# TheShadow29/zsgnet-pytorch

Measured on AMD Instinct MI355X. Metric: train images/sec, higher is better.
Workload: dtype f32

## Files before the change

### zsgnet-pytorch_amd/csrc/common.h

```cpp
#pragma once
#include <hip/hip_runtime.h>
#include <hip/hip_ext.h>
#include <stdint.h>
#include <stdio.h>
#include <string.h>

#include "zsg.h"

typedef float f32x4 __attribute__((ext_vector_type(4)));
typedef float f32x16 __attribute__((ext_vector_type(16)));

struct BnbDev {
    const float* x;
    const float* mean;
    const float* invstd;
    const unsigned char* mask;
    int store_masked;
};

int zsg_conv_pw_launch(const zsg_conv_desc* d, int uw, const float* src, const float* wt, float* out, const float* bias, const float* add_src,
                       const float* mask_src, float* bn_partials, const BnbDev* bnb, hipStream_t st);

bool zsg_conv_mx_ok(const zsg_conv_desc* d, const char** why);
int zsg_conv_mx_groups(const zsg_conv_desc* d);
int zsg_conv_mx_launch(const zsg_conv_desc* d, const float* src, const float* wt, float* out, const float* bias, const float* add_src,
                       const float* mask_src, float* bn_partials, hipStream_t st);

#ifndef ZSG_MAIN_PRIO
#define ZSG_MAIN_PRIO 3
#endif
typedef int (*zsg_prio_setter_t)(int);
void zsg_register_prio_setter(zsg_prio_setter_t fn);
#define ZSG_DEFINE_PRIO_FLAG()                                                                                                      \
    __constant__ int zsg_prio_flag_c = ZSG_MAIN_PRIO;                                                                               \
    static int zsg_prio_set_(int v) {                                                                                               \
        return hipMemcpyToSymbol(HIP_SYMBOL(zsg_prio_flag_c), &v, sizeof(int), 0, hipMemcpyHostToDevice) == hipSuccess ? 0 : -3;      \
    }                                                                                                                               \
    namespace {                                                                                                                     \
    struct ZsgPrioReg {                                                                                                             \
        ZsgPrioReg() { zsg_register_prio_setter(zsg_prio_set_); }                                                                   \
    } zsg_prio_reg_;                                                                                                                \
    }
#define ZSG_SET_MAIN_PRIO() do { if (zsg_prio_flag_c) __builtin_amdgcn_s_setprio(3); } while (0)

#define ZSG_WAVE 64
#define ZSG_NUM_CU 256
#define ZSG_NUM_XCD 8
#define ZSG_MAX_DEV 64

void zsg_set_error(const char* fmt, ...);
#define ZSG_FAIL(code, ...)          \
    do {                             \
        zsg_set_error(__VA_ARGS__);  \
        return (code);               \
    } while (0)
#define ZSG_REQUIRE(cond, ...)                   \
    do {                                         \
        if (!(cond)) ZSG_FAIL(-1, __VA_ARGS__);  \
    } while (0)
#define ZSG_CHECK_LAUNCH(name)                                                            \
    do {                                                                                  \
        hipError_t e__ = hipGetLastError();                                               \
        if (e__ != hipSuccess) ZSG_FAIL(-3, "%s: launch failed: %s", name, hipGetErrorString(e__)); \
    } while (0)

extern thread_local hipEvent_t zsg_tls_completion_event;
extern thread_local int zsg_tls_completion_uses;
#define ZSG_LAUNCH(kernel, grid, block, shmem, stream, ...)                                                                   \
    do {                                                                                                                      \
        if (zsg_tls_completion_event) {                                                                                       \
            hipExtLaunchKernelGGL(kernel, grid, block, shmem, stream, nullptr, zsg_tls_completion_event, 0, __VA_ARGS__);      \
            ++zsg_tls_completion_uses;                                                                                        \
        } else                                                                                                                  \
            hipLaunchKernelGGL(kernel, grid, block, shmem, stream, __VA_ARGS__);                                              \
    } while (0)

#define ZSG_SK_FLAG_BYTES 16384
#define ZSG_SK_ERR_WORD (ZSG_SK_FLAG_BYTES / 4 - 1)
void* zsg_stream_workspace(hipStream_t st, size_t* bytes);

struct ZsgProfScope {
    int slot;
    hipStream_t st;
    ZsgProfScope(const char* name, hipStream_t s, double flops, double bytes);
    ~ZsgProfScope();
};
extern int g_zsg_prof_on;
extern int g_zsg_deterministic;
#define ZSG_PROF(name, stream, flops, bytes) ZsgProfScope prof__(name, (hipStream_t)(stream), (flops), (bytes))

static inline double zsg_conv_alg_bytes(const zsg_conv_desc* d, bool reads_out) {
    double e = (double)d->N * d->seg[0].ty.n * d->seg[0].tx.n * d->C;
    for (int s = 0; s < d->nseg; ++s) {
        const zsg_seg& a = d->seg[s];
        e += (double)d->B * a.src_H * a.src_W * d->C + (double)d->B * a.rows_y * a.rows_x * d->N * (reads_out ? 2.0 : 1.0);
    }
    return 4.0 * e;
}

__device__ __forceinline__ float wave_sum(float v) {
#pragma unroll
    for (int o = 32; o > 0; o >>= 1) v += __shfl_xor(v, o, 64);
    return v;
}
__device__ __forceinline__ double wave_sum_d(double v) {
#pragma unroll
    for (int o = 32; o > 0; o >>= 1) v += __shfl_xor(v, o, 64);
    return v;
}
// ... 28 lines not shown
```

### zsgnet-pytorch_amd/csrc/wgrad.hip

```cpp
#include <stdlib.h>

#include "wgrad_common.h"

template <int KL>
__device__ __forceinline__ void wgrad_reduce_body(const WgReduceJob& p, int block, f32x4* sm_) {
    constexpr int EL = 256 / KL;
    f32x4 (*sm)[EL] = (f32x4 (*)[EL])sm_;
    const int q4 = p.ncols / 4;
    const int64_t total = (int64_t)p.N * q4;
    const size_t slab = (size_t)p.N * p.ncols;
    const int el = threadIdx.x % EL, kl = threadIdx.x / EL;
    const int64_t i = (int64_t)block * EL + el;
    f32x4 s = {0.f, 0.f, 0.f, 0.f};
    int n = 0, q = 0;
    if (i < total) {
        n = (int)(i / q4);
        q = (int)(i % q4) * 4;
        const float* src = p.ws + (size_t)n * p.ncols + q;
#pragma unroll 4
        for (int k = kl; k < p.splits; k += KL) s += *(const f32x4*)(src + k * slab);
    }
    sm[kl][el] = s;
    __syncthreads();
    for (int o = KL / 2; o > 0; o >>= 1) {
// ... 156 lines not shown
        for (int j = 0; j < NB; ++j) *(f32x4*)&Bs[buf][kb + PB * j][4 * gb] = rb[j];
    };

    f32x16 acc[TM][TN];
#pragma unroll
    for (int i = 0; i < TM; ++i)
#pragma unroll
        for (int j = 0; j < TN; ++j)
#pragma unroll
            for (int e = 0; e < 16; ++e) acc[i][j][e] = 0.f;

    const int n_kt = kt_end - kt_begin;
    if (n_kt > 0) {
        load_tile(ra[0], rb[0], true);
        store_tile(0, ra[0], rb[0]);
#pragma unroll
        for (int st = 0; st < NS - 1; ++st) load_tile(ra[st], rb[st], n_kt > st + 1);
    }
    __syncthreads();

    const int am = wm * (32 * TM) + TM * li;
    const int bn = wn * (32 * TN) + TN * li;
    auto k_step = [&](int it, f32x4 (&cur_a)[NA], f32x4 (&cur_b)[NB], f32x4 (&nxt_a)[NA], f32x4 (&nxt_b)[NB]) {
        const int buf = it & 1;
        load_tile(nxt_a, nxt_b, it + NS < n_kt);
        __builtin_amdgcn_sched_barrier(0);
#pragma unroll
        for (int kk = 0; kk < WG_BK / 2; ++kk) {
            const int k = 2 * kk + lh;
            float fa[TM], fb[TN];
#pragma unroll
            for (int i = 0; i < TM; ++i) fa[i] = As[buf][k][am + i];
#pragma unroll
            for (int j = 0; j < TN; ++j) fb[j] = Bs[buf][k][bn + j];
#pragma unroll
            for (int i = 0; i < TM; ++i)
#pragma unroll
                for (int j = 0; j < TN; ++j)
                    acc[i][j] = __builtin_amdgcn_mfma_f32_32x32x2f32(fa[i], fb[j], acc[i][j], 0, 0, 0);
        }
        store_tile(buf ^ 1, cur_a, cur_b);
        __syncthreads();
    };
    for (int it = 0; it < n_kt; it += NS) {
#pragma unroll
        for (int st = 0; st < NS; ++st)
            if (it + st < n_kt) k_step(it + st, ra[st], rb[st], ra[(st + NS - 1) % NS], rb[(st + NS - 1) % NS]);
    }
    if (kt_begin >= kt_end) return;

#pragma unroll
    for (int j = 0; j < TN; ++j) {
        const int qc = n0 + wn * (32 * TN) + TN * li + j;
        const bool cok = qc < p.ncols;
        size_t coff;
        if (p.ws) {
            coff = (size_t)split * p.N * p.ncols + qc;
        } else {
            const int qq = cok ? qc : 0;
            const int tapi = qq / p.C;
            const int c = qq - tapi * p.C;
            const int jy = tapi / p.txn, jx = tapi - jy * p.txn;
            const int wr = p.ty.w0 + jy * p.ty.wstep, ws_ = p.tx.w0 + jx * p.tx.wstep;
            coff = (size_t)((wr * p.wS + ws_) * p.wC + p.wc0 + c);
        }
        const int ld = p.ws ? p.ncols : p.wt_ld;
        float* dst = p.ws ? p.ws : p.dw;
#pragma unroll
        for (int i = 0; i < TM; ++i) {
#pragma unroll
            for (int e = 0; e < 16; ++e) {
                const int n = m0 + wm * (32 * TM) + TM * ((e & 3) + 8 * (e >> 2) + 4 * lh) + i;
                if (cok && n < p.N) {
                    float* o = dst + (size_t)n * ld + coff;
                    *o = (!p.ws && p.accumulate) ? *o + acc[i][j][e] : acc[i][j][e];
                }
            }
        }
    }
}

extern "C" size_t zsg_conv_wgrad_workspace_bytes(const zsg_conv_desc* d) {
    if (!d) return 0;
    int splits = (d->tile_hint >> 16) & 0xff;
    if (splits <= 0) splits = 64;
    const size_t ncols = (size_t)d->seg[0].ty.n * d->seg[0].tx.n * d->C;
    return (size_t)splits * d->N * ncols * sizeof(float);
}

static const int g_zsg_wg_no_dense = [] { const char* e = getenv("ZSG_WG_DENSE"); return (e && e[0] == '0') ? 1 : 0; }();

static int conv_wgrad_impl(const zsg_conv_desc* d, const float* src, const float* dy, float* dw, int32_t accumulate, void* ws,
                           size_t ws_bytes, void* stream) {
    ZSG_REQUIRE(d && src && dy && dw, "conv_wgrad: null argument");
    ZSG_REQUIRE(d->nseg >= 1 && d->nseg <= ZSG_MAX_SEG, "conv_wgrad: nseg=%d", d->nseg);
    ZSG_REQUIRE(d->C > 0 && (d->C % 4) == 0 && (d->src_ld % 4) == 0 && (d->wC % 4) == 0 && (d->wc0 % 4) == 0,
                "conv_wgrad: C=%d src_ld=%d wC=%d wc0=%d must be multiples of 4", d->C, d->src_ld, d->wC, d->wc0);
    WgParams p;
    memset(&p, 0, sizeof(p));
    p.src = src; p.dy = dy; p.dw = dw; p.accumulate = accumulate ? 1 : 0;
    p.C = d->C; p.N = d->N; p.src_ld = d->src_ld; p.out_ld = d->out_ld; p.wS = d->wS; p.wC = d->wC; p.wc0 = d->wc0;
    p.wt_ld = d->wt_ld; p.nseg = d->nseg;
    p.ty = d->seg[0].ty; p.tx = d->seg[0].tx;
    p.txn = p.tx.n;
    p.ncols = p.ty.n * p.tx.n * d->C;
    int kt = 0;
    double rows_all = 0;
    bool wide = false;
    const bool avec = (d->out_ld & 3) == 0;
    int BKsel = (avec && ((d->tile_hint >> 25) & 1) && ((d->tile_hint >> 8) & 0xff) != 255) ? 32 : 16;
    for (int s = 0; s < d->nseg; ++s)
        if (d->seg[s].src_bstride >= (1 << 23) || d->seg[s].out_bstride >= (1 << 23)) BKsel = 16;
    p.bk = BKsel;
    for (int s = 0; s < d->nseg; ++s) {
        const zsg_seg& a = d->seg[s];
        ZSG_REQUIRE(memcmp(&a.ty, &p.ty, sizeof(zsg_taps)) == 0 && memcmp(&a.tx, &p.tx, sizeof(zsg_taps)) == 0,
                    "conv_wgrad: segments must share one tap structure (pass the forward descriptor)");
        const int64_t rows = (int64_t)d->B * a.rows_y * a.rows_x;
        ZSG_REQUIRE(rows > 0 && rows < (1ll << 24), "conv_wgrad: seg %d rows=%lld (must be < 2^24)", s, (long long)rows);
        ZSG_REQUIRE(a.src_off + (int64_t)d->B * a.src_bstride < (1ll << 29) && a.out_off + (int64_t)d->B * a.out_bstride < (1ll << 29),
                    "conv_wgrad: tensor exceeds 2^29 elements (2 GB window)");
        ZSG_REQUIRE((a.src_off % 4) == 0 && (a.src_bstride % 4) == 0, "conv_wgrad: seg %d source not 16-byte aligned", s);
        ZSG_REQUIRE(d->src_ld < (1 << 23) && d->out_ld < (1 << 23) && (int64_t)a.src_H * a.src_W < (1 << 23) &&
                        (int64_t)(a.rows_y * a.osy + a.opy + 1) * a.out_W < (1 << 23),
                    "conv_wgrad: seg %d: a row pitch / per-image pixel count exceeds 2^23", s);
        if (a.src_bstride >= (1 << 23) || a.out_bstride >= (1 << 23)) wide = true;
        WgSegDev& o = p.seg[s];
        o.rows_y = a.rows_y; o.rows_x = a.rows_x; o.rows = (int)rows; o.kt0 = kt;
        o.src_H = a.src_H; o.src_W = a.src_W; o.sy = a.sy; o.sx = a.sx;
        o.out_W = a.out_W; o.osy = a.osy; o.osx = a.osx; o.opy = a.opy; o.opx = a.opx;
        o.src_off = (int)a.src_off; o.src_bstride = (int)a.src_bstride;
        o.out_off = (int)a.out_off; o.out_bstride = (int)a.out_bstride;
        o.inv_per = 1.0f / (float)(a.rows_y * a.rows_x);
        o.inv_rx = 1.0f / (float)a.rows_x;
        kt += cdiv(rows, BKsel);
        rows_all += (double)rows;
    }
    p.kt_total = kt;
    bool dense = avec && !wide && p.ty.n == 1 && p.tx.n == 1 && p.ty.d0 == 0 && p.tx.d0 == 0 && !g_zsg_wg_no_dense;
    for (int s = 0; s < d->nseg && dense; ++s) {
        const zsg_seg& a = d->seg[s];
        dense = a.sy == 1 && a.sx == 1 && a.osy == 1 && a.osx == 1 && a.opy == 0 && a.opx == 0 && a.rows_y == a.src_H && a.rows_x == a.src_W &&
                a.out_W == a.rows_x && a.src_bstride == (int64_t)a.src_H * a.src_W * d->src_ld &&
                a.out_bstride == (int64_t)a.rows_y * a.rows_x * d->out_ld;
    }
    int TM = (d->N > 64) ? 2 : 1;
    int TN = (p.ncols > 64) ? 2 : 1;
    int want_splits = 0, w8 = 0;
    if (d->tile_hint) {
        TM = ((d->tile_hint & 0xff) >= 128) ? 2 : 1;
        TN = (((d->tile_hint >> 8) & 0xff) >= 128) ? 2 : 1;
        if (((d->tile_hint >> 8) & 0xff) == 255 && TM == 1) TN = 4;
        want_splits = (d->tile_hint >> 16) & 0xff;
        w8 = ((d->tile_hint >> 24) & 1) && TM == 2 && TN == 2;
    }
    if (!avec || wide) { TM = 1; TN = 1; w8 = 0; }
    p.m_tiles = cdiv(d->N, 64 * TM);
    p.n_tiles = cdiv(p.ncols, 64 * TN);
    const int nmn = p.m_tiles * p.n_tiles;
    int splits = want_splits > 0 ? want_splits : (2 * ZSG_NUM_CU + nmn - 1) / nmn;
    if (splits > 64 && want_splits <= 0) splits = 64;
    if (splits > kt / 2) splits = kt / 2;
    if (splits < 1) splits = 1;
    p.kt_chunk = cdiv(kt, splits);
    p.splits = cdiv(kt, p.kt_chunk);
    if (p.splits > 1) {
        const size_t need = (size_t)p.splits * d->N * p.ncols * sizeof(float);
        if (!ws || ws_bytes < need) ZSG_FAIL(-2, "conv_wgrad: workspace too small (%zu < %zu bytes)", ws_bytes, need);
        p.ws = (float*)ws;
    }
    hipStream_t st = (hipStream_t)stream;
    int dev = 0;
    (void)hipGetDevice(&dev);
    ZSG_REQUIRE(dev >= 0 && dev < ZSG_MAX_DEV, "conv_wgrad: device %d", dev);
    const double wg_flops = 2.0 * rows_all * d->N * p.ncols;
    const double wg_bytes = zsg_conv_alg_bytes(d, accumulate != 0);
    dim3 grid(nmn * p.splits);
// ... 58 lines not shown
```

### zsgnet-pytorch_amd/mdl.py

```python
import ctypes as _ct
import math
import os
import struct as _struct
import types
import weakref
from dataclasses import dataclass, field
from typing import Any, Dict, List, Optional, Tuple

import numpy as np
import torch
from torch import nn

from . import anchors as anchors_mod
from ._lib import check, lib, require_gpu, stream_ptr
from .ops import (Level, Program, TView, WinoJobs, apply_main_priority_env, autotune_conv, autotune_wgrad_batch, conv_out, ensure_stream_scratch, dgrad_desc, fwd_desc, igemm_partial_rows, marshal,
                  shared_side_stream, tile_hint, wino_mode, wino_ok)
from .params import ParamStore, pad4, register_named

VGG_BASE = [64, 64, "M", 128, 128, "M", 256, 256, 256, "C", 512, 512, 512, "M", 512, 512, 512]
SSD_EXTRAS = [256, "S", 512, 128, "S", 256, 128, 256, 128, 256]

WGRAD_DTYPES = ("fp32", "bf16")
EVAL_TTAS = ("none", "flip")
EVAL_DTYPES = ("fp32", "bf16", "bf16_act")
# ... 1238 lines not shown
        if self.training:
            y = self.conv(L, x, name=yname or (L.name + ".y"), bn_fuse=Lb)
            return self.bn(Lb, y, relu, residual=residual, name=name)
        net = self.net
        n_w = L.cout * L.k * L.k * L.cpad
        w_off = self.fold_used
        b_off = w_off + (n_w + 3) // 4 * 4
        self.fold_used = b_off + (L.cout + 3) // 4 * 4
        assert self.fold_used <= self.fold_arena.numel(), "BN-fold arena too small"
        ents = net.store.entries
        self.fold_jobs.append((ents[L.name + ".weight"].offset, w_off, ents[Lb.name + ".weight"].offset, ents[Lb.name + ".bias"].offset,
                               b_off, self.fold_rows, L.cout, L.k * L.k * L.cpad, Lb.index))
        self.fold_rows += L.cout
        lv = x.levels[0]
        out = self.act(name or Lb.name, x.B, conv_out(lv.H, L.k, L.stride, L.pad, L.dil), conv_out(lv.W, L.k, L.stride, L.pad, L.dil), L.cout,
                       dtype=torch.float32 if L.merge_x else self.adt)
        d = fwd_desc(x, out, L.cpad, L.cout, L.k, L.stride, L.pad, L.dil, wC=L.cpad, relu=relu, merge_x=L.merge_x)
        wt, bias = self.fold_arena[w_off:w_off + n_w], self.fold_arena[b_off:b_off + L.cout]
        args = (x.buf, wt, out.buf, bias, residual.buf if residual is not None else None, None, None)
        if self._bf16_conv(d, x.buf, wt, L.cpad, 0, out.buf, bias, args[4], L.name + "+bn"):
            return out
        if x.b16 or out.b16 or (residual is not None and residual.b16):
            x32, o32, r32, finish = self._via_f32(x, out, residual)
            args = (x32.buf, wt, o32.buf, bias, r32.buf if r32 is not None else None, None, None)
            x, real_out, out = x32, out, o32
        else:
            real_out, finish = out, (lambda: None)
        wargs = None
        if wino_ok(L.k, L.stride, L.pad, L.dil) and not L.merge_x and wino_mode() != "0":
            U, job = self._wino_u(wt.data_ptr(), L.cout, L.cpad, L.k * L.k * L.cpad, L.cpad, 0)
            wargs = (x.buf, U) + args[2:]
        self._tune("igemm", lib.zsg_conv_igemm, d, args, stream_ptr(), wino_args=wargs)
        if d.use_wino:
            self.wino_jobs["fwd"].add(*job)
            self.fwd.add(lib.zsg_conv_wino, d, *wargs, what=L.name + "+bn")
        else:
            self.fwd.add(lib.zsg_conv_igemm, d, *args, what=L.name + "+bn")
        finish()
        return real_out

    def _wt(self, L: ConvL, cred: int) -> torch.Tensor:
        if L.name not in self.wt:
            n = L.cpad * L.k * L.k * cred
            off = self.wt_arena_used
            self.wt_arena_used += (n + 3) // 4 * 4
            assert self.wt_arena_used <= self.wt_arena.numel(), "dgrad weight arena too small"
            self.wt[L.name] = self.wt_arena[off:off + n]
            e = self.net.store.entries[L.name + ".weight"]
            self.wt_jobs.append((e.offset, off, L.cout, L.k * L.k, L.cpad, cred))
            check(lib.zsg_transpose_w(self.net.store.flat.data_ptr() + 4 * e.offset, self.wt[L.name].data_ptr(), L.cout, L.k * L.k, L.cpad, cred,
                                      stream_ptr()), "transpose_w")
        return self.wt[L.name]

    def _finish_prep(self):
        import struct
        if not self.wt_jobs:
            return
        blob, tile0 = b"", 0
        for (so, do, N, T, Cc, ld) in self.wt_jobs:
            tc, tn = (Cc + 63) // 64, (ld + 63) // 64
            assert Cc % 4 == 0 and ld % 4 == 0 and so % 4 == 0 and do % 4 == 0
            blob += struct.pack("<qqiiiiiiii", so, do, N, T, Cc, ld, tile0, tc, tn, 0)
            tile0 += T * tc * tn
        self.wt_jobs_dev = torch.frombuffer(bytearray(blob), dtype=torch.uint8).to(self.dev)
        self.prep.add(lib.zsg_transpose_w_batched, self.net.store.flat, self.wt_arena, self.wt_jobs_dev, len(self.wt_jobs), tile0,
                      what="transpose all dgrad weight images")
        if self.dpack_jobs:
            blob = b"".join(_struct.pack("<qqiiiiiiii", *j) for j in self.dpack_jobs)
            self.dpack_jobs_dev = torch.frombuffer(bytearray(blob), dtype=torch.uint8).to(self.dev)
            self.prep.add(lib.zsg_pack_w_bf16_batched, self.dpack_jobs_dev, len(self.dpack_jobs), self.dpack_blocks,
                          what="pack bf16 dgrad weight images")
        wj = self.wino_jobs["bwd"]
        if wj.jobs:
            self.prep.add(lib.zsg_wino_weights, wj.finish(self.dev), len(wj.jobs), wj.blocks, what="wino dgrad filter transforms")

    def _conv_rg(self, L: ConvL, src: Act) -> bool:
        return src.requires_grad or self.trains(L.name + ".weight") or (L.bias and self.trains(L.name + ".bias"))

    def _conv_bwd(self, L: ConvL, src: Act, out: Act, dy: Optional[Act] = None, completes_bn: bool = False):
        dy = dy or out.grad
        if dy is None:
            return
        if self.trains(L.name + ".weight"):
            dw = fwd_desc(src, dy, L.cpad, L.cout, L.k, L.stride, L.pad, L.dil, wC=L.cpad)
            self.wgrad(dw, src, dy, L.name + ".weight", "wgrad:" + L.name, merge_x=L.merge_x)
        if L.bias and self.trains(L.name + ".bias"):
            base = dy.levels[0].off
            self.bwd.add(lib.zsg_colsum, dy.buf[base:], 1, 0, dy.rows(), dy.ld, 0, L.cout, self.G(L.name + ".bias"), 1,
                         what="bgrad:" + L.name, lane=1)
        if src.requires_grad:
            self.dgrad(L, dy, src, n=L.cpad, completes_bn=completes_bn)

    def wgrad(self, d, src: Act, dy: Act, pname: str, what: str, merge_x: bool = False):
        gw = self.G(pname)
        args = (src.buf, dy.buf, gw, 1, self.wg_ws, self.wg_ws_bytes)
        targs = (src.buf, dy.buf, self.tune_dw, 0, self.wg_ws, self.wg_ws_bytes)
        s0 = d.seg[0]
        wino = (d.wR == 3 and d.wS == 3 and s0.sy == 1 and s0.ty.d0 == -1 and s0.ty.dstep == 1 and not d.merge_x
                and dy.ld % 4 == 0 and wino_mode() != "0")
        if self.wgrad_bf16 and self._wgrad_bf16_ok(d, merge_x):
            self._tune("wgrad", lib.zsg_conv_wgrad_bf16, d, targs, stream_ptr(), self.wg_ws_bytes)
            self.bwd.add(lib.zsg_conv_wgrad_bf16, d, *args, what=what + "+bf16", lane=1)
            self._wg_log.append((len(self.bwd.calls) - 1, d, src, dy, gw, pname, what + "+bf16"))
            return
        self._tune("wgrad", lib.zsg_conv_wgrad, d, targs, stream_ptr(), self.wg_ws_bytes, wino_args=targs if wino else None)
        self.bwd.add(lib.zsg_conv_wgrad_wino if d.use_wino else lib.zsg_conv_wgrad, d, *args, what=what, lane=1)
        self._wg_log.append((len(self.bwd.calls) - 1, d, src, dy, gw, pname, what))

    @staticmethod
    def _wgrad_bf16_ok(d, merge_x: bool = False) -> bool:
        dq = type(d).from_buffer_copy(d)
        dq.merge_x = int(bool(merge_x))
        return bool(lib.zsg_conv_wgrad_bf16_supported(_ct.byref(dq)))

    def dgrad(self, L: ConvL, dy: Act, src: Act, n: int, row0: int = 0, dx: Optional[Act] = None, completes_bn: bool = False):
        cred = dy.ld
        assert cred % 4 == 0
        wt = self._wt(L, cred)
        dx = dx or self.grad_of(src)
        d = dgrad_desc(dy, dx, cred, n, L.k, L.stride, L.pad, L.dil)
        wt_off = row0 * L.k * L.k * cred
        if d.zero_fill and not dx.gfilled:
            (self.prep if self._side_prep else self.bwd).add(lib.zsg_memset_f32, self.base(dx), sum(dx.B * l.H * l.W * dx.ld for l in dx.levels), 0.0,
                                                             what="zero:" + L.name)
            dx.gfilled = True
        mask = None
        if src.needs_mask:
            deltas = {sl.off - dl.off for sl, dl in zip(src.levels, dx.levels)}
            assert len(deltas) == 1 and src.ld == dx.ld, "ReLU mask needs one common offset between src and its gradient"
            mask = src.buf.data_ptr() + 4 * deltas.pop()
            self.bwd.keep.append(src.buf)
        if self._b16_eligible(L.name) and not getattr(src, "bn_out", False) and lib.zsg_conv_igemm_bf16_m_supported(_ct.byref(d)):
            key = (L.name, row0, n)
            if key not in self._dpack:
                self._dpack[key], job, nblk = self._pack_image(wt.data_ptr() + 4 * wt_off, n, L.k * L.k, cred, 0, cred)
                self.dpack_jobs.append(job + (self.dpack_blocks, 0))
                self.dpack_blocks += nblk
            add = dx if dx.gfilled else None
            args = (dy.buf, self._dpack[key], dx.buf, None, dx.buf if dx.gfilled else None, mask)
            self._tune("igemm", lib.zsg_conv_igemm_bf16_m, d, args, stream_ptr())
            self.bwd.add(lib.zsg_conv_igemm_bf16_m, d, *args, what="dgrad:" + L.name + "+bf16")
            self._b16_log.append(dict(kind="dgrad", what="dgrad:" + L.name, idx=-1, call=self.bwd.calls[-1], d=type(d).from_buffer_copy(d),
                                      src=dy, out=dx, add=add, mask=src if mask is not None else None, pname=L.name + ".weight",
                                      window=(row0, n)))
            dx.gfilled = True
            dx.last_writer = None
            return
        if self._encb_eligible(L) and lib.zsg_conv_igemm_bf16_m_supported(_ct.byref(d)):
            key = (L.name, row0, n)
            if key not in self._dpack:
                self._dpack[key], job, nblk = self._pack_image(wt.data_ptr() + 4 * wt_off, n, L.k * L.k, cred, 0, cred)
                self.dpack_jobs.append(job + (self.dpack_blocks, 0))
                self.dpack_blocks += nblk
            add = dx if dx.gfilled else None
            args = (dy.buf, self._dpack[key], dx.buf, None, dx.buf if dx.gfilled else None, mask)
            autotune_conv("igemm", lib.zsg_conv_igemm_bf16_m, d, args, stream_ptr())
            self.bwd.add(lib.zsg_conv_igemm_bf16_m, d, *args, what="dgrad:" + L.name + "+bf16")
            self._b16_log.append(dict(kind="enc_dgrad", what="dgrad:" + L.name, idx=-1, call=self.bwd.calls[-1], d=type(d).from_buffer_copy(d),
                                      src=dy, out=dx, add=add, mask=src if mask is not None else None, pname=L.name + ".weight",
                                      window=(row0, n), bn=None))
            dx.gfilled = True
            covers_all = not d.zero_fill and mask is None and d.tile_hint and dx.ld == n and n % 4 == 0
            dx.last_writer = (len(self.bwd.calls) - 1, d, args, "dgrad:" + L.name + "+bf16", self._b16_log[-1]) if covers_all else None
            return
        args = (dy.buf, wt[wt_off:], dx.buf, None, dx.buf if dx.gfilled else None, mask, None)
        wargs = None
        if wino_ok(L.k, L.stride, L.pad, L.dil) and wino_mode() != "0":
# ... 1236 lines not shown
```

### zsgnet-pytorch_amd/ops.py

```python
import ctypes as C
import os
from dataclasses import dataclass, field
from typing import List, Optional, Sequence, Tuple

import torch

from ._lib import ConvDesc, Seg, Taps, lib, check, ZSG_MAX_SEG, ZsgError


@dataclass
class Level:
    off: int
    H: int
    W: int
    bstride: int


@dataclass
class TView:
    buf: torch.Tensor
    B: int
    C: int
    ld: int
    levels: List[Level]
# ... 679 lines not shown
            for target in (256, 384, 512, 768, 1024, 2048):
                sp = max(1, min(target // nmn, rows // 64, 255))
                if sp not in seen and sp * N * ncols * 4 <= ws_bytes:
                    seen.add(sp)
                    cands.append(tile_hint(bm, bn, sp))
    return cands


def autotune_conv(kind: str, fn, d: ConvDesc, args: Sequence, stream: int, ws_bytes: int = 0, split_penalty_ms: float = 0.0,
                  wino_args: Optional[Sequence] = None, wino_fn=None, allow_sk: bool = True) -> int:
    d.use_wino = False
    mode = wino_mode() if wino_args is not None else "0"
    if mode == "0":
        wino_args = None
    no_tune = os.environ.get("ZSG_AUTOTUNE", "1") == "0" or not torch.cuda.is_available()
    if wino_args is not None and (mode == "force" and no_tune):
        d.tile_hint, d.use_wino = (wino_default_hint(d) if kind == "igemm" else 0), True
        return d.tile_hint | WINO_FLAG
    if no_tune:
        return 0
    _check_table_arch()
    io = fn is lib.zsg_conv_igemm_bf16_io
    bf16m = fn is lib.zsg_conv_igemm_bf16_m
    bf16bn = fn is lib.zsg_conv_igemm_bf16_bn
    bf16 = io or bf16m or bf16bn or fn is lib.zsg_conv_igemm_bf16
    add_src, mask = (args[4], args[5] if (bf16m or not bf16) else None) if (kind == "igemm" and not bf16bn) else (None, None)
    key = _sig(kind, d, (add_src is not None, mask is not None, add_src is not None and add_src is args[2], split_penalty_ms > 0,
                         mode if wino_args is not None else "", deterministic(), "bf16" if bf16 else "fp32",
                         fn.__name__ + (":io%d" % args[5] if io else ""),
                         os.environ.get("ZSG_PW", "1") != "0" and not (d.merge_x and os.environ.get("ZSG_MX", "1") == "0"),
                         allow_sk and os.environ.get("ZSG_SK", "1") != "0"))
    d._tune_key = key
    if key in _TUNE_CACHE:
        v = _TUNE_CACHE[key]
        d.tile_hint, d.use_wino = v & ~WINO_FLAG, bool(v & WINO_FLAG)
        return v
    rows = sum(d.B * d.seg[i].rows_y * d.seg[i].rows_x for i in range(d.nseg))
    cands = []
    if bf16:
        cands = [tile_hint(64, 64, 1), tile_hint(128, 64, 1)] + ([tile_hint(128, 128, 1)] if d.N > 64 else [])
    elif kind == "igemm":
        tiles = [(64, 64), (128, 64)] + ([(128, 128)] if d.N > 64 else [])
        s0 = d.seg[0]
        dense = (d.nseg == 1 and not d.relu and d.out_ld == d.N and s0.osy == 1 and s0.osx == 1 and s0.out_W == s0.rows_x
                 and s0.out_bstride == s0.rows_y * s0.rows_x * d.N)
        for bm, bn in tiles:
            cands.append(tile_hint(bm, bn, 1))
            if not d.merge_x and (bm == 128 or bn == 64):
                cands.append(tile_hint(bm, bn, 1, 1))
        if not d.merge_x and d.C % 64 == 0 and os.environ.get("ZSG_K64", "1") != "0":
            cands += [tile_hint(bm, bn, 1, w8) | K64_FLAG for bm, bn in tiles for w8 in (0, 1) if not (bm == 128 and bn == 128 and not w8)]
        if fn is lib.zsg_conv_igemm and os.environ.get("ZSG_PW", "1") != "0" and not (d.merge_x and os.environ.get("ZSG_MX", "1") == "0"):
            cands += pw_cands(d)
        if allow_sk and fn is not lib.zsg_conv_igemm_bnpre:
            ensure_stream_scratch(stream)
            cands += sk_cands(d, rows)
        blocks64 = ((rows + 63) // 64) * ((d.N + 63) // 64)
        n_it = s0.ty.n * s0.tx.n * ((d.C + 31) // 32)
        if dense and blocks64 < 1024 and not deterministic():
            for sp in (2, 3, 4, 6, 8, 12, 16, 24, 32):
                if sp <= n_it and blocks64 * sp <= 3072:
                    cands.append(tile_hint(64, 64, sp))
                    if d.C % 64 == 0 and 2 * sp <= n_it and os.environ.get("ZSG_K64", "1") != "0":
                        cands.append(tile_hint(64, 64, sp, 1) | K64_FLAG)
                    if blocks64 * sp < 256:
                        cands.append(tile_hint(128, 64, sp))
    elif fn is lib.zsg_conv_wgrad_bf16:
        cands = wgrad_bf16_cands(d.N, d.seg[0].ty.n * d.seg[0].tx.n * d.C, rows, ws_bytes)
    else:
        ncols = d.seg[0].ty.n * d.seg[0].tx.n * d.C
        for bm in ((64, 128) if d.N > 64 else (64,)):
            for bn in (((64, 128) if ncols > 64 else (64,)) + ((255,) if (bm == 64 and d.N <= 64 and 128 < ncols <= 256 and d.out_ld % 4 == 0) else ())):
                nmn = ((d.N + bm - 1) // bm) * ((ncols + (256 if bn == 255 else bn) - 1) // (256 if bn == 255 else bn))
                seen = set()
                for target in (256, 384, 512, 768, 1024, 2048):
                    sp = max(1, min(target // nmn, rows // 64, 255))
                    if sp not in seen and sp * d.N * ncols * 4 <= ws_bytes:
                        seen.add(sp)
                        cands.append(tile_hint(bm, bn, sp))
                        if bm == 128 and bn == 128:
                            cands.append(tile_hint(bm, bn, sp, 0, 1))
                            cands.append(tile_hint(bm, bn, sp, 1, 0))
                            cands.append(tile_hint(bm, bn, sp, 1, 1))
    trials = [] if mode == "force" else [(fn, marshal(fn, (d,) + tuple(args)), h, 0) for h in cands]
    if wino_args is not None and kind == "igemm":
        wfn = wino_fn or lib.zsg_conv_wino
        wconv = marshal(wfn, (d,) + tuple(wino_args))
        if allow_sk:
            ensure_stream_scratch(stream)
        trials += [(wfn, wconv, h, WINO_FLAG) for h in _wino_cands(d, allow_sk)]
    elif wino_args is not None:
        wconv = marshal(lib.zsg_conv_wgrad_wino, (d,) + tuple(wino_args))
        tiles = sum(d.B * ((d.seg[i].src_H + 1) // 2) * ((d.seg[i].src_W + 1) // 2) for i in range(d.nseg))
        nmn = ((d.N + 63) // 64) * ((d.C + 63) // 64)
        seen = set()
        for target in (128, 192, 256, 384, 512, 768):
            sp = max(1, min(target // nmn, tiles // 16, 255))
            if sp not in seen and sp * d.N * 9 * d.C * 4 <= ws_bytes:
                seen.add(sp)
                trials.append((lib.zsg_conv_wgrad_wino, wconv, tile_hint(64, 64, sp), WINO_FLAG))
                if sp > 1 and nmn * sp >= 128:
                    trials.append((lib.zsg_conv_wgrad_wino, wconv, tile_hint(64, 64, sp, 1), WINO_FLAG))
    def set_hint(h):
        d.tile_hint = h

    snap = args[2].clone() if (kind == "igemm" and isinstance(add_src, torch.Tensor) and add_src is args[2]) else None
    best = _pick_best(trials, set_hint, stream, lambda h: split_penalty_ms if (kind == "igemm" and ((h >> 16) & 0xff) > 1) else 0.0)
    if snap is not None:
        args[2].copy_(snap)
    if os.environ.get("ZSG_TUNE_VERIFY") and fn in (lib.zsg_conv_igemm, lib.zsg_conv_wgrad, lib.zsg_conv_igemm_bf16_m):
        _verify_candidates(kind, key, trials, set_hint, args[2], args[4] if kind == "igemm" else None, stream)
    d.tile_hint, d.use_wino = best & ~WINO_FLAG, bool(best & WINO_FLAG)
    _TUNE_CACHE[key] = best
    _TUNE_ALTS[key] = list(_LAST_RANKING)
    global _TUNE_DIRTY
    _TUNE_DIRTY = True
    TUNE_INFO["tuned_now"] += 1
    return best


def autotune_wgrad_batch(d: ConvDesc, njobs: int, wino: bool, srcs, dys, scratch_dw: torch.Tensor, ws: torch.Tensor, ws_bytes: int, stream: int) -> int:
    global _TUNE_DIRTY
    key = _sig("wgradb", d, (njobs, bool(wino), deterministic()))
    if key in _TUNE_CACHE:
        d.tile_hint = _TUNE_CACHE[key]
        return d.tile_hint
    assert wino, "job batches exist for the Winograd weight gradient only (the direct kernel's measured no gain in the step: profiles/r06_wgrad_batching.txt)"
    fn = lib.zsg_conv_wgrad_wino_batched
    VP = C.c_void_p * njobs
    a_src, a_dy, a_dw = VP(*[t.data_ptr() for t in srcs]), VP(*[t.data_ptr() for t in dys]), VP(*([scratch_dw.data_ptr()] * njobs))
    conv = (C.byref(d), C.c_int32(njobs), C.cast(a_src, C.c_void_p), C.cast(a_dy, C.c_void_p), C.cast(a_dw, C.c_void_p), C.c_int32(0),
            C.c_void_p(ws.data_ptr()), C.c_size_t(ws_bytes))
    trials, seen = [], set()
    if wino:
        tiles = sum(d.B * ((d.seg[i].src_H + 1) // 2) * ((d.seg[i].src_W + 1) // 2) for i in range(d.nseg))
        nmn = ((d.N + 63) // 64) * ((d.C + 63) // 64) * njobs
        for target in (128, 192, 256, 384, 512, 768):
            sp = max(1, min(target // nmn, tiles // 16, 255))
            if sp not in seen and njobs * sp * d.N * 9 * d.C * 4 <= ws_bytes:
                seen.add(sp)
                trials.append((fn, conv, tile_hint(64, 64, sp), 0))

    def set_hint(h):
        d.tile_hint = h
    best = _pick_best(trials, set_hint, stream, lambda h: 0.0)
    if not best:
        raise ZsgError(f"wgrad batch: no candidate ran ({lib.zsg_last_error().decode()})")
    d.tile_hint = best
    _TUNE_CACHE[key] = best
    _TUNE_DIRTY = True
    TUNE_INFO["tuned_now"] += 1
    return best


REFINE_WINDOW = float(os.environ.get("ZSG_REFINE_WINDOW", "1.08"))
REFINE_WINDOW_WAVES = float(os.environ.get("ZSG_REFINE_WINDOW_WAVES", "1.30"))
REFINE_NOISE = float(os.environ.get("ZSG_REFINE_NOISE", "0.003"))


def hint_compatible(d: ConvDesc, kind: str, cur: int, alt: int) -> bool:
    if (cur ^ alt) & WINO_FLAG:
        return False
    hc, ha = cur & ~WINO_FLAG, alt & ~WINO_FLAG
    if kind == "wgrad":
        return True
    if ((hc >> 16) & 0xff) > 1 or ((ha >> 16) & 0xff) > 1:
# ... 63 lines not shown
```

Before: 1234.

## Add streaming MFMA weight-gradient kernel for merge_x first-layer convolutions

```diff
diff --git a/zsgnet-pytorch_amd/csrc/common.h b/zsgnet-pytorch_amd/csrc/common.h
--- a/zsgnet-pytorch_amd/csrc/common.h
+++ b/zsgnet-pytorch_amd/csrc/common.h
@@ -25,6 +25,9 @@
 int zsg_conv_mx_groups(const zsg_conv_desc* d);
 int zsg_conv_mx_launch(const zsg_conv_desc* d, const float* src, const float* wt, float* out, const float* bias, const float* add_src,
                        const float* mask_src, float* bn_partials, hipStream_t st);
+int zsg_conv_mxwg_groups(const zsg_conv_desc* d);
+int zsg_conv_mxwg_launch(const zsg_conv_desc* d, const float* src, const float* dy, float* dw, int accumulate, void* ws, size_t ws_bytes,
+                         hipStream_t st);
 
 #ifndef ZSG_MAIN_PRIO
 #define ZSG_MAIN_PRIO 3
diff --git a/zsgnet-pytorch_amd/csrc/mxwg.hip b/zsgnet-pytorch_amd/csrc/mxwg.hip
--- /dev/null
+++ b/zsgnet-pytorch_amd/csrc/mxwg.hip
@@ -0,0 +1,206 @@
+#include "wgrad_common.h"
+
+#define MXWG_WAVES 8
+#define MXWG_N 64
+#define MXWG_WINDOW 0x40000000u
+#define MXWG_OOB 0x40000000u
+
+typedef float f32x2 __attribute__((ext_vector_type(2)));
+
+struct MxwgParams {
+    const float* src;
+    const float* dy;
+    float* ws;
+    int M;
+    int per_img, rows_x;
+    float inv_per, inv_rx;
+    int src_H, src_W, sy, sx, d0y, d0x, dy_step;
+    int TX;
+    int src_off, src_bstride;
+    int src_bias;
+    int out_off, out_ld;
+    int units;
+};
+
+template <int R, int R0, int RW, int TXS>
+__device__ __forceinline__ void mxwg_stream(const MxwgParams& p, f32x16 (&acc)[2][3], int first, int stride, int lane) {
+    const int li = lane & 31, lh = lane >> 5;
+    const rsrc_t rs = __builtin_amdgcn_make_buffer_rsrc((char*)const_cast<float*>(p.src) - p.src_bias, 0, MXWG_WINDOW, 0x00020000);
+    const int M = p.M, srcH = p.src_H, srcW = p.src_W, out_ld = p.out_ld;
+    const int kx = li % TXS, rr = li / TXS;
+    const int lane_off = 16 * kx + (R0 + rr) * (16 * p.dy_step * srcW);
+    const int need = (rr < RW) ? ((1 << (8 + R0 + rr)) | (1 << kx)) : (1 << 30);
+    const int lane_dy = 4 * (lh * out_ld + 2 * li);
+    const int lane_bp = 4 * lh;
+
+    auto decode = [&](int u, int& org, int& bits) {
+        const int m = u * 32 + li;
+        const bool ok = m < M;
+        const int mm = ok ? m : 0;
+        const int b = fdiv(mm, p.per_img, p.inv_per);
+        const int rem = mm - b * p.per_img;
+        const int y = fdiv(rem, p.rows_x, p.inv_rx);
+        const int x = rem - y * p.rows_x;
+        const int xs = x * p.sx + p.d0x, ys = y * p.sy + p.d0y;
+        org = 4 * (p.src_off + b * p.src_bstride) + 16 * (ys * srcW + xs) + p.src_bias;
+        int v = 0;
+#pragma unroll
+        for (int r = 0; r < R; ++r) v |= ((unsigned)(ys + r * p.dy_step) < (unsigned)srcH) ? (1 << (8 + r)) : 0;
+#pragma unroll
+        for (int k = 0; k < TXS; ++k) v |= ((k < p.TX) & ((unsigned)(xs + k) < (unsigned)srcW)) ? (1 << k) : 0;
+        bits = ok ? v : 0;
+    };
+    f32x2 D[8];
+    f32x4 P[8];
+#define MXWG_REQUEST(u, h, s, org, bits)                                                                                      \
+    {                                                                                                                         \
+        const int a__ = __builtin_amdgcn_ds_bpermute(lane_bp + 4 * (16 * (h) + 2 * (s)), org) + lane_off;                     \
+        const int mb__ = __builtin_amdgcn_ds_bpermute(lane_bp + 4 * (16 * (h) + 2 * (s)), bits);                              \
+        const int m__ = (u) * 32 + 16 * (h) + 2 * (s);                                                                        \
+        const int left__ = __builtin_amdgcn_readfirstlane(min(max(M - m__, 0), 2));             \
+        const rsrc_t rd__ = make_rsrc_n(p.dy + p.out_off + (size_t)(left__ ? m__ : 0) * out_ld, 4u * left__ * out_ld);        \
+        D[s] = __builtin_bit_cast(f32x2, __builtin_amdgcn_raw_buffer_load_b64(rd__, lane_dy, 0, 0));                          \
+        P[s] = buf_load4(rs, ((mb__ & need) == need) ? (unsigned)a__ : MXWG_OOB);                                             \
+    }
+    int u = first, org_c, bits_c, org_n, bits_n;
+    decode(u, org_c, bits_c);
+#pragma unroll
+    for (int s = 0; s < 8; ++s) MXWG_REQUEST(u, 0, s, org_c, bits_c);
+    for (; u < p.units; u += stride) {
+        const int un = u + stride;
+        decode(un, org_n, bits_n);
+#pragma unroll
+        for (int h = 0; h < 2; ++h) {
+#pragma unroll
+            for (int s = 0; s < 8; ++s) {
+#pragma unroll
+                for (int c = 0; c < 3; ++c) {
+                    acc[0][c] = __builtin_amdgcn_mfma_f32_32x32x2f32(D[s][0], P[s][c], acc[0][c], 0, 0, 0);
+                    acc[1][c] = __builtin_amdgcn_mfma_f32_32x32x2f32(D[s][1], P[s][c], acc[1][c], 0, 0, 0);
+                }
+                __builtin_amdgcn_sched_barrier(0);
+                if (h == 0) MXWG_REQUEST(u, 1, s, org_c, bits_c) else MXWG_REQUEST(un, 0, s, org_n, bits_n)
+                __builtin_amdgcn_sched_barrier(0);
+            }
+        }
+        org_c = org_n;
+        bits_c = bits_n;
+    }
+#undef MXWG_REQUEST
+}
+
+template <int R>
+__global__ __launch_bounds__(64 * MXWG_WAVES) void mxwg_kernel(const MxwgParams p) {
+    constexpr int SLOTS = (R == 7) ? 4 : MXWG_WAVES;
+    constexpr int TXS = (R == 7) ? 8 : 4;
+    extern __shared__ __attribute__((aligned(16))) float red[];
+    const int tid = threadIdx.x, lane = tid & 63, wave = __builtin_amdgcn_readfirstlane(tid >> 6);
+    const int li = lane & 31, lh = lane >> 5;
+    const int slot = wave % SLOTS;
+    const int r0 = (R == 7 && wave >= 4) ? 4 : 0, rw = (R == 7) ? (wave >= 4 ? 3 : 4) : R;
+    const int G = (int)gridDim.x;
+
+    f32x16 acc[2][3];
+#pragma unroll
+    for (int n = 0; n < 2; ++n)
+#pragma unroll
+        for (int c = 0; c < 3; ++c)
+#pragma unroll
+            for (int e = 0; e < 16; ++e) acc[n][c][e] = 0.f;
+    const int first = (int)blockIdx.x + G * slot;
+    if (R == 7) {
+        if (wave < 4) mxwg_stream<7, 0, 4, TXS>(p, acc, first, G * SLOTS, lane);
+        else mxwg_stream<7, 4, 3, TXS>(p, acc, first, G * SLOTS, lane);
+    } else {
+        mxwg_stream<R, 0, R, TXS>(p, acc, first, G * SLOTS, lane);
+    }
+
+    const int TX = p.TX, ncols = R * TX * 4;
+    const int kx = li % TXS, rr = li / TXS;
+    const bool lane_col = (kx < TX) & (rr < rw);
+    const int col = ((r0 + rr) * TX + kx) * 4;
+    for (int round = 0; round < SLOTS; ++round) {
+        if (slot == round && lane_col) {
+#pragma unroll
+            for (int j = 0; j < 2; ++j)
+#pragma unroll
+                for (int e = 0; e < 16; ++e) {
+                    float* q = red + (2 * ((e & 3) + 8 * (e >> 2) + 4 * lh) + j) * ncols + col;
+#pragma unroll
+                    for (int c = 0; c < 3; ++c) q[c] = round ? q[c] + acc[j][c][e] : acc[j][c][e];
+                    if (round == 0) q[3] = 0.f;
+                }
+        }
+        __syncthreads();
+    }
+    float* slab = p.ws + (size_t)blockIdx.x * MXWG_N * ncols;
+    for (int idx = tid; idx < MXWG_N * ncols / 4; idx += 64 * MXWG_WAVES) *(f32x4*)(slab + 4 * idx) = *(const f32x4*)(red + 4 * idx);
+}
+
+
+int zsg_conv_mxwg_groups(const zsg_conv_desc* d) {
+    const int64_t rows = (int64_t)d->B * d->seg[0].rows_y * d->seg[0].rows_x;
+    const int slots = d->seg[0].ty.n == 7 ? 4 : MXWG_WAVES;
+    const int g = cdiv(cdiv(rows, 32), slots);
+    return g < ZSG_NUM_CU ? g : ZSG_NUM_CU;
+}
+
+template <int R>
+static int mxwg_launch(const MxwgParams& p, int grid, hipStream_t st, double flops, double bytes, const char* kname) {
+    const size_t lds = (size_t)MXWG_N * R * 8 * 4 * sizeof(float);
+    static bool attr_done[ZSG_MAX_DEV] = {};
+    int dev = 0;
+    (void)hipGetDevice(&dev);
+    ZSG_REQUIRE(dev >= 0 && dev < ZSG_MAX_DEV, "conv_wgrad: device %d", dev);
+    if (!attr_done[dev]) {
+        hipError_t e = hipFuncSetAttribute((const void*)mxwg_kernel<R>, hipFuncAttributeMaxDynamicSharedMemorySize, (int)lds);
+        if (e != hipSuccess) ZSG_FAIL(-3, "conv_wgrad: hipFuncSetAttribute: %s", hipGetErrorString(e));
+        attr_done[dev] = true;
+    }
+    ZSG_PROF(kname, st, flops, bytes);
+    ZSG_LAUNCH((mxwg_kernel<R>), dim3(grid), dim3(64 * MXWG_WAVES), lds, st, p);
+    return 0;
+}
+
+int zsg_conv_mxwg_launch(const zsg_conv_desc* d, const float* src, const float* dy, float* dw, int accumulate, void* ws, size_t ws_bytes,
+                         hipStream_t st) {
+    const char* why = "";
+    ZSG_REQUIRE(zsg_conv_mx_ok(d, &why), "conv_wgrad: the streaming first-layer kernel (tile_hint BM = 32, merge_x) needs %s", why);
+    const zsg_seg& s = d->seg[0];
+    const int64_t rows = (int64_t)d->B * s.rows_y * s.rows_x;
+    ZSG_REQUIRE(d->out_ld >= MXWG_N, "conv_wgrad: the streaming first-layer kernel needs dY rows of 64 channels");
+    ZSG_REQUIRE(rows < (1ll << 24) && (int64_t)s.rows_y * s.rows_x < (1ll << 23),
+                "conv_wgrad: the streaming first-layer kernel needs fewer than 2^24 pixels (2^23 per image)");
+    ZSG_REQUIRE((((uintptr_t)src | (uintptr_t)dy | (uintptr_t)dw | (uintptr_t)ws) & 15) == 0,
+                "conv_wgrad: the streaming first-layer kernel needs 16-byte aligned operands");
+    const int grid = zsg_conv_mxwg_groups(d);
+    const int ncols = s.ty.n * s.tx.n * d->C;
+    const size_t need = (size_t)grid * d->N * ncols * sizeof(float);
+    if (!ws || ws_bytes < need) ZSG_FAIL(-2, "conv_wgrad: workspace too small (%zu < %zu bytes)", ws_bytes, need);
+    MxwgParams p;
+    memset(&p, 0, sizeof(p));
+    p.src = src; p.dy = dy; p.ws = (float*)ws;
+    p.M = (int)rows;
+    p.per_img = s.rows_y * s.rows_x; p.rows_x = s.rows_x;
+    p.inv_per = 1.0f / (float)p.per_img; p.inv_rx = 1.0f / (float)p.rows_x;
+    p.src_H = s.src_H; p.src_W = s.src_W; p.sy = s.sy; p.sx = s.sx; p.d0y = s.ty.d0; p.d0x = s.tx.d0; p.dy_step = s.ty.dstep;
+    p.TX = s.tx.n;
+    p.src_off = (int)s.src_off; p.src_bstride = (int)s.src_bstride;
+    p.out_off = (int)s.out_off; p.out_ld = d->out_ld;
+    p.units = cdiv(p.M, 32);
+    const int64_t org0 = 16 * ((int64_t)s.ty.d0 * s.src_W + s.tx.d0);
+    p.src_bias = org0 < 0 ? (int)-org0 : 0;
+    ZSG_REQUIRE(4 * (s.src_off + (int64_t)d->B * s.src_bstride) + p.src_bias < (int64_t)MXWG_WINDOW, "conv_wgrad: the streaming first-layer kernel needs a source below 2^30 bytes");
+    const double flops = 2.0 * (double)rows * d->N * ncols;
+    const double bytes = zsg_conv_alg_bytes(d, accumulate != 0);
+    int rc;
+    if (s.ty.n == 7) rc = mxwg_launch<7>(p, grid, st, flops, bytes, "mxwg_kernel<7>");
+    else if (s.ty.n == 3) rc = mxwg_launch<3>(p, grid, st, flops, bytes, "mxwg_kernel<3>");
+    else ZSG_FAIL(-1, "conv_wgrad: the streaming first-layer kernel is built for 7x7 and 3x3 windows (%dx%d)", s.ty.n, s.tx.n);
+    if (rc) return rc;
+    WgReduceJob j;
+    wg_reduce_job_fill(j, d, p.ws, dw, accumulate, grid);
+    wg_reduce_launch(j, st);
+    ZSG_CHECK_LAUNCH("conv_wgrad");
+    return 0;
+}
diff --git a/zsgnet-pytorch_amd/csrc/wgrad.hip b/zsgnet-pytorch_amd/csrc/wgrad.hip
--- a/zsgnet-pytorch_amd/csrc/wgrad.hip
+++ b/zsgnet-pytorch_amd/csrc/wgrad.hip
@@ -262,6 +262,8 @@
 
 extern "C" size_t zsg_conv_wgrad_workspace_bytes(const zsg_conv_desc* d) {
     if (!d) return 0;
+    if (d->merge_x && (d->tile_hint & 0xff) == 32)
+        return zsg_conv_mx_ok(d, nullptr) ? (size_t)zsg_conv_mxwg_groups(d) * d->N * d->seg[0].ty.n * d->seg[0].tx.n * d->C * sizeof(float) : 0;
     int splits = (d->tile_hint >> 16) & 0xff;
     if (splits <= 0) splits = 64;
     const size_t ncols = (size_t)d->seg[0].ty.n * d->seg[0].tx.n * d->C;
@@ -273,6 +275,8 @@
 static int conv_wgrad_impl(const zsg_conv_desc* d, const float* src, const float* dy, float* dw, int32_t accumulate, void* ws,
                            size_t ws_bytes, void* stream) {
     ZSG_REQUIRE(d && src && dy && dw, "conv_wgrad: null argument");
+    if (d->merge_x && (d->tile_hint & 0xff) == 32)
+        return zsg_conv_mxwg_launch(d, src, dy, dw, accumulate, ws, ws_bytes, (hipStream_t)stream);
     ZSG_REQUIRE(d->nseg >= 1 && d->nseg <= ZSG_MAX_SEG, "conv_wgrad: nseg=%d", d->nseg);
     ZSG_REQUIRE(d->C > 0 && (d->C % 4) == 0 && (d->src_ld % 4) == 0 && (d->wC % 4) == 0 && (d->wc0 % 4) == 0,
                 "conv_wgrad: C=%d src_ld=%d wC=%d wc0=%d must be multiples of 4", d->C, d->src_ld, d->wC, d->wc0);
diff --git a/zsgnet-pytorch_amd/mdl.py b/zsgnet-pytorch_amd/mdl.py
--- a/zsgnet-pytorch_amd/mdl.py
+++ b/zsgnet-pytorch_amd/mdl.py
@@ -1344,7 +1344,8 @@
         if dy is None:
             return
         if self.trains(L.name + ".weight"):
-            dw = fwd_desc(src, dy, L.cpad, L.cout, L.k, L.stride, L.pad, L.dil, wC=L.cpad)
+            dw = fwd_desc(src, dy, L.cpad, L.cout, L.k, L.stride, L.pad, L.dil, wC=L.cpad,
+                          merge_x=L.merge_x and not wino_ok(L.k, L.stride, L.pad, L.dil))
             self.wgrad(dw, src, dy, L.name + ".weight", "wgrad:" + L.name, merge_x=L.merge_x)
         if L.bias and self.trains(L.name + ".bias"):
             base = dy.levels[0].off
diff --git a/zsgnet-pytorch_amd/ops.py b/zsgnet-pytorch_amd/ops.py
--- a/zsgnet-pytorch_amd/ops.py
+++ b/zsgnet-pytorch_amd/ops.py
@@ -785,6 +785,11 @@
                             cands.append(tile_hint(bm, bn, sp, 0, 1))
                             cands.append(tile_hint(bm, bn, sp, 1, 0))
                             cands.append(tile_hint(bm, bn, sp, 1, 1))
+        if d.merge_x and os.environ.get("ZSG_MX", "1") != "0":
+            keep, d.tile_hint = d.tile_hint, tile_hint(32, 64, 1)
+            if 0 < lib.zsg_conv_wgrad_workspace_bytes(C.byref(d)) <= ws_bytes:
+                cands.append(d.tile_hint)
+            d.tile_hint = keep
     trials = [] if mode == "force" else [(fn, marshal(fn, (d,) + tuple(args)), h, 0) for h in cands]
     if wino_args is not None and kind == "igemm":
         wfn = wino_fn or lib.zsg_conv_wino
```

New measurement: 1238 (median of 6 runs). About the same (+0.3%).
